# NIRVANALAN/LN3Diff

Hardware: AMD Instinct MI355X
Metric: 3D samples/sec (250-step DiT-L/2 + 256^2 triplane render) (higher is better)
Workload: dtype bf16; 1 GPU; BASELINE configs[1]: DiT-L/2 text-cond T23D, EulerEDM/LegacyDDPM-sigma 250 steps, CFG 6.5 (network batch 2B), batch 8 per GPU, VAE decode DiT2-L/2 + conv decoder, 40 views @ 256^2 (64+64 samples/ray); global_batch=8, views=40, res=256, parallelism=dp1 (independent samples per rank, no in-loop collective)

## Files before the change

### ln3diff_amd/csrc/gemm_bf16.hip

```cpp
#include <stdlib.h>
#include "common.h"
#include "../../include/ln3d.h"

#define BMF 128
#define BTK 128
#define BK 64
#define ROWB 144
#define TILEB (128 * ROWB)
#define GEMM_LDS (4 * TILEB)

#include "gemm_epi.h"

template <int EPI>
__global__ __launch_bounds__(256) void gemm_bf16_kernel(GemmP p) {
  extern __shared__ __attribute__((aligned(16))) char smem[];
  const int tid = threadIdx.x, lane = tid & 63, wid = tid >> 6;
  const int wf = wid >> 1, wt = wid & 1;
  const int l31 = lane & 31, hi = lane >> 5;

  const int nft = (p.N + BMF - 1) / BMF;
  const int ft = blockIdx.x % nft, tt = blockIdx.x / nft;
  const int f0 = ft * BMF, t0 = tt * BTK;

  const int c = tid & 7, r0 = tid >> 3;
  const bf16_t* wsrc[4]; const bf16_t* xsrc[4];
#pragma unroll
  for (int i = 0; i < 4; ++i) {
    int rf = f0 + r0 + 32 * i; rf = rf < p.N ? rf : p.N - 1;
    int rt = t0 + r0 + 32 * i; rt = rt < p.M ? rt : p.M - 1;
    wsrc[i] = p.W + (int64_t)rf * p.ldw + c * 8;
    xsrc[i] = p.X + (int64_t)rt * p.ldx + c * 8;
  }
  const int st_off = r0 * ROWB + c * 16;

  f32x16 acc[2][2];
#pragma unroll
  for (int i = 0; i < 2; ++i)
#pragma unroll
    for (int j = 0; j < 2; ++j)
#pragma unroll
      for (int r = 0; r < 16; ++r) acc[i][j][r] = 0.f;

  uint4 ra[4], rb[4];
  const int nk = p.K / BK;
#pragma unroll
  for (int i = 0; i < 4; ++i) {
    ra[i] = *reinterpret_cast<const uint4*>(wsrc[i]);
    rb[i] = *reinterpret_cast<const uint4*>(xsrc[i]);
  }
#pragma unroll
  for (int i = 0; i < 4; ++i) {
    *reinterpret_cast<uint4*>(smem + st_off + i * 32 * ROWB) = ra[i];
    *reinterpret_cast<uint4*>(smem + TILEB + st_off + i * 32 * ROWB) = rb[i];
  }
  __syncthreads();

  const int a_off = (wf * 64 + l31) * ROWB + hi * 16;
  const int b_off = TILEB + (wt * 64 + l31) * ROWB + hi * 16;

  auto mma_tile = [&](const char* base) {
#pragma unroll
    for (int ks = 0; ks < 4; ++ks) {
      bf16x8 a[2], b[2];
#pragma unroll
      for (int i = 0; i < 2; ++i) {
        a[i] = *reinterpret_cast<const bf16x8*>(base + a_off + i * 32 * ROWB + ks * 32);
        b[i] = *reinterpret_cast<const bf16x8*>(base + b_off + i * 32 * ROWB + ks * 32);
      }
#pragma unroll
      for (int i = 0; i < 2; ++i)
#pragma unroll
        for (int j = 0; j < 2; ++j)
          acc[i][j] = __builtin_amdgcn_mfma_f32_32x32x16_bf16(a[i], b[j], acc[i][j], 0, 0, 0);
    }
  };

  for (int kt = 0; kt + 1 < nk; ++kt) {
    const int buf = kt & 1;
    const int koff = (kt + 1) * BK;
    const uint4 na0 = *reinterpret_cast<const uint4*>(wsrc[0] + koff);
    const uint4 na1 = *reinterpret_cast<const uint4*>(wsrc[1] + koff);
    const uint4 na2 = *reinterpret_cast<const uint4*>(wsrc[2] + koff);
    const uint4 na3 = *reinterpret_cast<const uint4*>(wsrc[3] + koff);
    const uint4 nx0 = *reinterpret_cast<const uint4*>(xsrc[0] + koff);
    const uint4 nx1 = *reinterpret_cast<const uint4*>(xsrc[1] + koff);
    const uint4 nx2 = *reinterpret_cast<const uint4*>(xsrc[2] + koff);
    const uint4 nx3 = *reinterpret_cast<const uint4*>(xsrc[3] + koff);
    __builtin_amdgcn_sched_barrier(0);
    mma_tile(smem + buf * 2 * TILEB);
    __builtin_amdgcn_sched_barrier(0);
    char* nb = smem + (buf ^ 1) * 2 * TILEB + st_off;
    *reinterpret_cast<uint4*>(nb + 0 * 32 * ROWB) = na0;
    *reinterpret_cast<uint4*>(nb + 1 * 32 * ROWB) = na1;
    *reinterpret_cast<uint4*>(nb + 2 * 32 * ROWB) = na2;
    *reinterpret_cast<uint4*>(nb + 3 * 32 * ROWB) = na3;
    *reinterpret_cast<uint4*>(nb + TILEB + 0 * 32 * ROWB) = nx0;
    *reinterpret_cast<uint4*>(nb + TILEB + 1 * 32 * ROWB) = nx1;
    *reinterpret_cast<uint4*>(nb + TILEB + 2 * 32 * ROWB) = nx2;
    *reinterpret_cast<uint4*>(nb + TILEB + 3 * 32 * ROWB) = nx3;
    __syncthreads();
  }
  mma_tile(smem + ((nk - 1) & 1) * 2 * TILEB);

#pragma unroll
  for (int j = 0; j < 2; ++j) {
    const int tok = t0 + wt * 64 + j * 32 + l31;
    if (tok >= p.M) continue;
#pragma unroll
    for (int i = 0; i < 2; ++i) {
#pragma unroll
      for (int g = 0; g < 4; ++g) {
        const int fb = f0 + wf * 64 + i * 32 + 8 * g + 4 * hi;
        if (fb < p.N)
          epilogue4<EPI>(p, tok, fb, acc[i][j][4 * g + 0], acc[i][j][4 * g + 1], acc[i][j][4 * g + 2], acc[i][j][4 * g + 3]);
      }
    }
  }
}



template <int EPI, int NW, int WGT, int NI, int NJ>
__global__ __launch_bounds__(NW * 64, (NW == 4 && NI * NJ <= 6) ? 2 : NW / 4) void gemm_bf16_ring64_kernel(GemmP p) {
  constexpr int WGF = NW / WGT, BF = 32 * NI * WGF, BT = 32 * NJ * WGT;
  constexpr int WB = BF * 128, STAGEB = (BF + BT) * 128, NPW = (BF + BT) / 8 / NW;
  static_assert((BF + BT) / 8 % NW == 0, "DMA instructions must divide evenly over the waves");
  constexpr int NM = NI * NJ, NR = NI + NJ;
  static_assert(NM >= NR, "one fragment read per MFMA slot");
  extern __shared__ __attribute__((aligned(16))) char smem[];
  const int tid = threadIdx.x, lane = tid & 63;
  const int wid = __builtin_amdgcn_readfirstlane(tid >> 6);
  const int wf = wid / WGT, wt = wid % WGT;
  const int l31 = lane & 31, hi = lane >> 5;

  const int nft = (p.N + BF - 1) / BF, ntt = (p.M + BT - 1) / BT;
  const int ntiles = nft * ntt;
  int ft, tt;
  {
    const int b = blockIdx.x, xcd = b & 7, slot = b >> 3;
    if ((ntt & 7) == 0 && (nft & 3) == 0) {
      const int rows = ntt >> 3;
      const int g = slot / (rows * 4), rem = slot - g * rows * 4;
      ft = g * 4 + (rem & 3);
      tt = xcd * rows + (rem >> 2);
    } else {
      const int q = ntiles >> 3, r = ntiles & 7;
      const int tile = (xcd < r ? xcd * (q + 1) : r * (q + 1) + (xcd - r) * q) + slot;
      ft = tile % nft; tt = tile / nft;
    }
  }
  const int f0 = ft * BF, t0 = tt * BT;

  constexpr int NPWW = BF / 8 / NW, NPWX = BT / 8 / NW;
  static_assert(BF / 8 % NW == 0 && BT / 8 % NW == 0 && NPWW + NPWX == NPW, "row groups of both operands divide evenly over the waves");
  const int r8 = lane >> 3;
  const char* const Wb = reinterpret_cast<const char*>(p.W + (int64_t)f0 * p.ldw);
  const char* const Xb = reinterpret_cast<const char*>(p.X + (int64_t)t0 * p.ldx);
  uint32_t soff[NPW];
#pragma unroll
  for (int q = 0; q < NPW; ++q) {
    const int rt = 8 * (q < NPWW ? wid * NPWW + q : wid * NPWX + (q - NPWW)) + r8;
    const int chunk = (lane & 7) ^ ((rt >> 1) & 7);
    if (q < NPWW) {
      int r = f0 + rt; r = r < p.N ? r : p.N - 1;
      soff[q] = (uint32_t)(((int64_t)(r - f0) * p.ldw + chunk * 8) * 2);
    } else {
      int r = t0 + rt; r = r < p.M ? r : p.M - 1;
      soff[q] = (uint32_t)(((int64_t)(r - t0) * p.ldx + chunk * 8) * 2);
    }
  }
  const int dW0 = wid * NPWW * 1024, dX0 = WB + wid * NPWX * 1024;
  const uint32_t lds0 = (uint32_t)(uintptr_t)(lds_void_t*)smem;
#define Y_ISSUE1(s, q)                                                                                        \
  lds_dma16_s(((q) < NPWW ? Wb : Xb) + (int64_t)(s) * 128, soff[q],                                           \
              lds0 + ((s) & 1) * STAGEB + ((q) < NPWW ? dW0 + (q) * 1024 : dX0 + ((q) - NPWW) * 1024))

  const int key = (l31 >> 1) & 7;
  const int a_row = (wf * 32 * NI + l31) * 128;
  const int b_row = WB + (wt * 32 * NJ + l31) * 128;
#define Y_RDA(s, ks, i) (*reinterpret_cast<const bf16x8*>(smem + ((s) & 1) * STAGEB + a_row + (i) * 4096 + (((2 * (ks) + hi) ^ key) << 4)))
#define Y_RDB(s, ks, j) (*reinterpret_cast<const bf16x8*>(smem + ((s) & 1) * STAGEB + b_row + (j) * 4096 + (((2 * (ks) + hi) ^ key) << 4)))

  f32x16 acc[NI][NJ];
#pragma unroll
  for (int i = 0; i < NI; ++i)
#pragma unroll
    for (int j = 0; j < NJ; ++j)
#pragma unroll
      for (int r = 0; r < 16; ++r) acc[i][j][r] = 0.f;

  bf16x8 a0[NI], b0[NJ], a1[NI], b1[NJ];
  const int ns = p.K / 64;

  constexpr int XK = 2 * STAGEB, XKH = 96 * 128;
  if constexpr (EPI == LN3D_EPI_CROSS_ATTN) {
    static_assert(NI == 2 && NJ == 3 && WGT == 2 && (NW == 8 || NW == 4), "one head (64 features) per wave row: 256x192 (8 waves) or 128x192 (4 waves) tile");
    const int bsmp = t0 / p.tokens;
    const int nrows8 = (p.ctx_keys + 7) >> 3;
    const bf16_t* kc = (const bf16_t*)p.out1 + ((int64_t)bsmp * p.heads + (f0 >> 6)) * p.ctx_pad * 64;
    for (int idx = wid; idx < WGF * nrows8; idx += NW) {
      const int hh = idx / nrows8, j = idx - hh * nrows8;
      const int r = 8 * j + (lane >> 3);
      const bf16_t* src_k = kc + ((int64_t)hh * p.ctx_pad + r) * 64 + (((lane & 7) ^ ((r >> 1) & 7)) << 3);
      lds_dma16_v(src_k, lds0 + XK + hh * XKH + j * 1024);
    }
  }

#pragma unroll
  for (int q = 0; q < NPW; ++q) Y_ISSUE1(0, q);
  if (ns > 1) { _Pragma("unroll") for (int q = 0; q < NPW; ++q) Y_ISSUE1(1, q); }
  if (ns > 1) { asm volatile("s_waitcnt vmcnt(%0)" ::"n"(NPW) : "memory"); }
  else { asm volatile("s_waitcnt vmcnt(0)" ::: "memory"); }
  __builtin_amdgcn_s_barrier();
#pragma unroll
  for (int i = 0; i < NI; ++i) a0[i] = Y_RDA(0, 0, i);
#pragma unroll
  for (int j = 0; j < NJ; ++j) b0[j] = Y_RDB(0, 0, j);

#define Y_MMA(FA, FB, n) acc[(n) / NJ][(n) % NJ] = __builtin_amdgcn_mfma_f32_32x32x16_bf16(FA[(n) / NJ], FB[(n) % NJ], acc[(n) / NJ][(n) % NJ], 0, 0, 0)
  constexpr int D1 = (NPW + 1) / 2;
  constexpr int NLATE = NPW - D1;
#define Y_PHASE(CA, CB, NA, NB, s2, ks2, LATE, sd, L0, L1)                                                \
  _Pragma("unroll") for (int n = 0; n < NM; ++n) {                                                        \
    Y_MMA(CA, CB, n);                                                                                     \
    if (n < NI) NA[n] = Y_RDA(s2, ks2, n);                                                                \
    else if (n < NR) NB[n - NI] = Y_RDB(s2, ks2, n - NI);                                                 \
    if (LATE) {                                                                                           \
      _Pragma("unroll") for (int d = (L0); d < (L1); ++d)                                                 \
          if ((d - (L0)) * NM / ((L1) - (L0) > 0 ? (L1) - (L0) : 1) == n) Y_ISSUE1(sd, d);                \
    }                                                                                                     \
    __builtin_amdgcn_sched_barrier(0);                                                                    \
  }
  static_assert(NM - 1 >= NR, "one fragment read per MFMA slot behind the barrier");
  constexpr int LH = D1 + (NLATE + 1) / 2;
#define Y_STAGE(s, PREV, FILL, MORE)                                                                      \
  {                                                                                                       \
    Y_PHASE(a0, b0, a1, b1, s, 1, (PREV) && NLATE > 0, (s) + 1, D1, LH);                                  \
    Y_PHASE(a1, b1, a0, b0, s, 2, (PREV) && NLATE > 0, (s) + 1, LH, NPW);                                 \
    Y_PHASE(a0, b0, a1, b1, s, 3, false, 0, 0, 0);                                                        \
    _Pragma("unroll") for (int n = 0; n < NM; ++n) {                                                      \
      Y_MMA(a1, b1, n);                                                                                   \
      if (MORE && n == 0) {                                                                               \
        asm volatile("s_waitcnt vmcnt(0)" ::: "memory");                                                  \
        __builtin_amdgcn_s_waitcnt(0xC07F);                                                               \
        __builtin_amdgcn_s_barrier();                                                                     \
      }                                                                                                   \
      if (MORE) {                                                                                         \
        if (n >= 1 && n - 1 < NI) a0[n - 1] = Y_RDA((s) + 1, 0, n - 1);                                   \
        else if (n >= 1 && n - 1 < NR) b0[n - 1 - NI] = Y_RDB((s) + 1, 0, n - 1 - NI);                    \
      }                                                                                                   \
      if (FILL) {                                                                                         \
        _Pragma("unroll") for (int d = 0; d < D1; ++d)                                                    \
            if (1 + d * (NM - 1) / D1 == n) Y_ISSUE1((s) + 2, d);                                         \
      }                                                                                                   \
      __builtin_amdgcn_sched_barrier(0);                                                                  \
    }                                                                                                     \
  }
  __builtin_amdgcn_s_waitcnt(0xC07F);
  int s = 0;
  if (ns >= 3) {
    Y_STAGE(0, false, true, true);
    for (s = 1; s + 2 < ns; ++s) Y_STAGE(s, true, true, true);
    Y_STAGE(s, true, false, true);
    ++s;
  } else if (ns == 2) {
    Y_STAGE(0, false, false, true);
    s = 1;
  }
  constexpr bool kPre = EPI == LN3D_EPI_GATE_RES && NW <= 8 && NI % 2 == 0 && NI * NJ <= 6;
  float4 xpre[8];
  RunEpi<EPI> re_pre;
  bool have_pre = false;
  if constexpr (kPre) {
    const int fw0 = f0 + wf * 32 * NI, tw0 = t0 + wt * 32 * NJ;
    const bool full = (tw0 + 32 * NJ <= p.M) && (fw0 + 32 * NI <= p.N) && !((p.gate || p.rb) && p.gate_rows < 32);
    if (__builtin_amdgcn_readfirstlane(full ? 1 : 0)) {
      have_pre = true;
      const int rrow = lane >> 4, rc = lane & 15;
      re_pre.init(p, fw0 + 4 * rc, __builtin_amdgcn_readfirstlane(tw0), 0, 0, 0);
      const float* base = (const float*)p.out0 + (int64_t)(tw0 + rrow) * p.ldo + fw0 + 4 * rc;
#pragma unroll
      for (int it = 0; it < 8; ++it) xpre[it] = *reinterpret_cast<const float4*>(base + (int64_t)(4 * it) * p.ldo);
    }
  }
  Y_STAGE(s, false, false, false);

  if constexpr (EPI == LN3D_EPI_CROSS_ATTN) {
    const int bsmp = t0 / p.tokens;
    const int nkb = (p.ctx_keys + 63) >> 6, nkt = (p.ctx_keys + 31) >> 5;
    __builtin_amdgcn_s_barrier();
    {
      const bf16_t* vc = (const bf16_t*)p.out2 + ((int64_t)bsmp * p.heads + (f0 >> 6)) * 64 * p.ctx_pad;
      for (int idx = wid; idx < WGF * nkb * 8; idx += NW) {
        const int hh = idx / (nkb * 8), rem = idx - hh * nkb * 8, kb = rem >> 3, j = rem & 7;
        const int vrow = 8 * j + (lane >> 3);
        const bf16_t* src_v = vc + ((int64_t)hh * 64 + vrow) * p.ctx_pad + kb * 64 + (((lane & 7) ^ ((vrow >> 1) & 7)) << 3);
        lds_dma16_v(src_v, lds0 + (hh * 2 + kb) * 8192 + j * 1024);
      }
    }
    const int kkey = (l31 >> 1) & 7;
    const char* kbase = smem + XK + wf * XKH + l31 * 128;
    float inv[NJ];
    uint32_t pk[NJ][24];
#pragma unroll
    for (int j = 0; j < NJ; ++j) {
      f32x16 st[3];
#pragma unroll
      for (int kt = 0; kt < 3; ++kt)
#pragma unroll
        for (int r = 0; r < 16; ++r) st[kt][r] = 0.f;
#pragma unroll
      for (int sd = 0; sd < 4; ++sd) {
        union { uint32_t u[4]; bf16x8 v; } qb;
#pragma unroll
        for (int jj = 0; jj < 4; ++jj)
          qb.u[jj] = pack2bf(acc[sd >> 1][j][8 * (sd & 1) + 2 * jj], acc[sd >> 1][j][8 * (sd & 1) + 2 * jj + 1]);
#pragma unroll
        for (int kt = 0; kt < 3; ++kt)
          if (kt < nkt) {
            const bf16x8 kf = *reinterpret_cast<const bf16x8*>(kbase + kt * 32 * 128 + (((2 * sd + hi) ^ kkey) << 4));
            st[kt] = __builtin_amdgcn_mfma_f32_32x32x16_bf16(kf, qb.v, st[kt], 0, 0, 0);
          }
      }
      float mx = -3.0e38f;
#pragma unroll
      for (int kt = 0; kt < 3; ++kt)
#pragma unroll
        for (int r = 0; r < 16; ++r) {
          const int key = kt * 32 + 4 * hi + (r & 3) + 8 * (r >> 2);
          st[kt][r] = key < p.ctx_keys ? st[kt][r] : -3.0e38f;
          mx = fmaxf(mx, st[kt][r]);
        }
      mx = fmaxf(mx, __shfl_xor(mx, 32, 64));
      const float m = mx * p.ctx_scale_log2;
      float psum = 0.f;
#pragma unroll
      for (int kt = 0; kt < 3; ++kt)
#pragma unroll
        for (int r = 0; r < 16; ++r) {
          const float pv = __builtin_amdgcn_exp2f(fmaf(st[kt][r], p.ctx_scale_log2, -m));
          st[kt][r] = pv;
          psum += pv;
        }
      inv[j] = 1.0f / (psum + __shfl_xor(psum, 32, 64));
#pragma unroll
      for (int ks = 0; ks < 6; ++ks)
#pragma unroll
        for (int jj = 0; jj < 4; ++jj)
          pk[j][4 * ks + jj] = pack2bf(st[ks >> 1][8 * (ks & 1) + 2 * jj], st[ks >> 1][8 * (ks & 1) + 2 * jj + 1]);
    }
    asm volatile("s_waitcnt vmcnt(0)" ::: "memory");
    __builtin_amdgcn_s_barrier();
    const char* vbase = smem + (wf * 2) * 8192 + l31 * 128;
#pragma unroll
    for (int j = 0; j < NJ; ++j) {
      f32x16 oa[2];
#pragma unroll
      for (int dt = 0; dt < 2; ++dt)
#pragma unroll
        for (int r = 0; r < 16; ++r) oa[dt][r] = 0.f;
#pragma unroll
      for (int ks = 0; ks < 6; ++ks)
        if (ks < 2 * nkt) {
          union { uint32_t u[4]; bf16x8 v; } pb;
#pragma unroll
          for (int jj = 0; jj < 4; ++jj) pb.u[jj] = pk[j][4 * ks + jj];
#pragma unroll
          for (int dt = 0; dt < 2; ++dt) {
            const bf16x8 vf = *reinterpret_cast<const bf16x8*>(vbase + (ks >> 2) * 8192 + dt * 32 * 128 + (((2 * (ks & 3) + hi) ^ kkey) << 4));
            oa[dt] = __builtin_amdgcn_mfma_f32_32x32x16_bf16(vf, pb.v, oa[dt], 0, 0, 0);
          }
        }
#pragma unroll
      for (int dt = 0; dt < 2; ++dt)
#pragma unroll
        for (int r = 0; r < 16; ++r) acc[dt][j][r] = oa[dt][r] * inv[j];
    }
  }
  bool direct = false;
  if constexpr (EPI == LN3D_EPI_HEADS) {
    direct = (p.transpose_mask != 0) && (f0 + BF > 2 * p.heads * p.head_dim);
    if constexpr (NI == 2) {
      const int dm = p.heads * p.head_dim;
      if ((p.head_dim & 7) == 0 && (dm & 63) == 0 && (p.tokens & 31) == 0 && (p.M % p.tokens) == 0 && (p.N % 64) == 0) {
        const int fw0 = f0 + wf * 64;
        const int which = fw0 / dm;
        const bool tr = fw0 < p.N && ((p.transpose_mask >> which) & 1);
        const int HD = p.head_dim, DP = p.head_dim_pad;
        __builtin_amdgcn_s_barrier();
        if (tr) {
          char* stg = smem + wid * 8192;
          bf16_t* dst = (bf16_t*)(which == 0 ? p.out0 : (which == 1 ? p.out1 : p.out2));
          const int fr = lane >> 2, c = lane & 3;
          int64_t vrow[4];
#pragma unroll
          for (int it = 0; it < 4; ++it) {
            const int fr_ = fw0 - which * dm + 16 * it + fr;
            const int hh_ = fr_ / HD;
            vrow[it] = (int64_t)hh_ * DP + (fr_ - hh_ * HD);
          }
#pragma unroll
          for (int j = 0; j < NJ; ++j) {
            const int tb = __builtin_amdgcn_readfirstlane(t0 + wt * 32 * NJ + j * 32);
            if (tb >= p.M) break;
            const int tp = (l31 & ~12) | ((l31 & 4) << 1) | ((l31 & 8) >> 1);
#pragma unroll
            for (int i = 0; i < 2; ++i)
#pragma unroll
              for (int g = 0; g < 4; ++g)
#pragma unroll
                for (int e = 0; e < 4; ++e)
                  *reinterpret_cast<float*>(stg + (i * 32 + 8 * g + 4 * hi + e) * 128 + tp * 4) = acc[i][j][4 * g + e];
            const int b = tb / p.tokens, t = tb - b * p.tokens;
#pragma unroll
            for (int it = 0; it < 4; ++it) {
              const int f = 16 * it + fr;
              const float bv = p.bias ? p.bias[fw0 + f] : 0.f;
              const float4 v0 = *reinterpret_cast<const float4*>(stg + f * 128 + c * 32);
              const float4 v1 = *reinterpret_cast<const float4*>(stg + f * 128 + c * 32 + 16);
              uint4 o;
              o.x = pack2bf(v0.x + bv, v0.y + bv); o.y = pack2bf(v0.z + bv, v0.w + bv);
              o.z = pack2bf(v1.x + bv, v1.y + bv); o.w = pack2bf(v1.z + bv, v1.w + bv);
              *reinterpret_cast<uint4*>(dst + ((int64_t)b * p.heads * DP + vrow[it]) * p.tok_pad + t + 8 * c) = o;
            }
          }
        } else if (fw0 < p.N) {
          char* stg = smem + wid * 8192;
          bf16_t* dst = (bf16_t*)(which == 0 ? p.out0 : (which == 1 ? p.out1 : p.out2));
          const int r8 = lane >> 3, c8 = lane & 7;
          const int fc_ = fw0 - which * dm + 8 * c8;
          const int h = fc_ / HD, d8 = fc_ - h * HD;
          float4 b0 = make_float4(0.f, 0.f, 0.f, 0.f), b1 = b0;
          if (p.bias) { b0 = *reinterpret_cast<const float4*>(p.bias + fw0 + 8 * c8); b1 = *reinterpret_cast<const float4*>(p.bias + fw0 + 8 * c8 + 4); }
          const float* nw = (HD == 64 && DP == 64) ? (which == 0 ? p.hn0 : (which == 1 ? p.hn1 : nullptr)) : nullptr;
          float4 n0 = make_float4(1.f, 1.f, 1.f, 1.f), n1 = n0;
          if (nw) { n0 = *reinterpret_cast<const float4*>(nw + 8 * c8); n1 = *reinterpret_cast<const float4*>(nw + 8 * c8 + 4); }
#pragma unroll
          for (int j = 0; j < NJ; ++j) {
// ... 111 lines not shown
  const int64_t jstride = (int64_t)32 * p.ldo * 2;
#define P_STORE(j, k) *reinterpret_cast<uint4*>(pbase + (j) * jstride + ((k) >> 1) * 64 + ((k) & 1) * 32) = pend[((j) - 1) * 8 + (k)]
#define P_STOREQ(q) P_STORE(1 + (q) / 8, (q) % 8)
#define P_PHASE(CB, NB, rslot, ks2, RD, LATE, WL, XL, dslot, L0, L1, SJ, ZERO, SYNC, FILL, WF, XF, fslot)  \
  _Pragma("unroll") for (int n = 0; n < NM; ++n) {                                                        \
    if (ZERO) { P_MMA0(af, CB, n); } else { P_MMA(af, CB, n); }                                           \
    if ((SYNC) && n == 0) {                                                                               \
      if ((SJ) >= 0 && have) { asm volatile("s_waitcnt vmcnt(3)" ::: "memory"); }                         \
      else { asm volatile("s_waitcnt vmcnt(0)" ::: "memory"); }                                           \
      __builtin_amdgcn_s_waitcnt(0xC07F);                                                                 \
      __builtin_amdgcn_s_barrier();                                                                       \
    }                                                                                                     \
    if (RD) {                                                                                             \
      if ((n & 3) == 3) af[n >> 2] = P_RDA(rslot, ks2, n >> 2);                                           \
      else if (n == 1 || n == 2) NB[n - 1] = P_RDB(rslot, ks2, n - 1);                                    \
      else if (n == 4 || n == 5) NB[n - 2] = P_RDB(rslot, ks2, n - 2);                                    \
    }                                                                                                     \
    if (LATE) {                                                                                           \
      _Pragma("unroll") for (int d = (L0); d < (L1); ++d)                                                 \
          if ((d - (L0)) * NM / ((L1) - (L0)) == n) P_ISSUE(WL, XL, dslot, d);                            \
    }                                                                                                     \
    if (FILL) {                                                                                           \
      _Pragma("unroll") for (int d = 0; d < D1; ++d)                                                      \
          if (1 + d * (NM - 1) / D1 == n) P_ISSUE(WF, XF, fslot, d);                                      \
    }                                                                                                     \
    if (!(SYNC) && (SJ) >= 0 && (n & 3) == 1 && n < 12) { if (have) P_STOREQ(3 * ((SJ) < 0 ? 0 : (SJ)) + (n >> 2)); } \
    __builtin_amdgcn_sched_barrier(0);                                                                    \
  }
#define P_STAGE(slot, LATE, WL, XL, WF, XF, SJ, ZERO, PRE)                                                \
  {                                                                                                       \
    P_PHASE(b0, b1, slot, 1, true, LATE, WL, XL, (slot) ^ 1, D1, LH, -1, ZERO, false, false, WF, XF, slot);      \
    P_PHASE(b1, b0, slot, 2, true, LATE, WL, XL, (slot) ^ 1, LH, NPW, -1, false, false, false, WF, XF, slot);    \
    P_PHASE(b0, b1, slot, 3, true, false, WL, XL, (slot) ^ 1, 0, 1, SJ, false, false, false, WF, XF, slot);      \
    P_PHASE(b1, b0, (slot) ^ 1, 0, PRE, false, WL, XL, (slot) ^ 1, 0, 1, SJ, false, true, true, WF, XF, slot);   \
  }

  f32x16 acc[NI][NJ];
  bf16x8 af[NI], b0[NJ], b1[NJ];
  const int ns = p.K / 64;
  const int64_t ldw2 = p.ldw * 2, ldx2 = p.ldx * 2;

  int vb = blockIdx.x, ft, tt;
  tile_of(vb, ft, tt);
  const char* Wc = reinterpret_cast<const char*>(p.W) + (int64_t)ft * BF * ldw2;
  const char* Xc = reinterpret_cast<const char*>(p.X) + (int64_t)tt * BT * ldx2;
  int par = 0;
#pragma unroll
  for (int q = 0; q < NPW; ++q) P_ISSUE(Wc, Xc, 0, q);
#pragma unroll
  for (int q = 0; q < NPW; ++q) P_ISSUE(Wc + 128, Xc + 128, 1, q);
  const uint32_t boff = (uint32_t)lane * 16;
  if (p.bias) { if (wid == 0) lds_dma16_s(p.bias + ft * BF, boff, lds0 + BIASB); }
  else if (wid < 2) *reinterpret_cast<float4*>(smem + BIASB + wid * 1024 + lane * 16) = make_float4(0.f, 0.f, 0.f, 0.f);
  asm volatile("s_waitcnt vmcnt(0)" ::: "memory");
  __builtin_amdgcn_s_barrier();
  __builtin_amdgcn_s_waitcnt(0xC07F);

  for (;;) {
    const int vbn = vb + G;
    const bool has_next = vbn < ntiles;
    int ftn, ttn;
    tile_of(has_next ? vbn : vb, ftn, ttn);
    const char* Wn = reinterpret_cast<const char*>(p.W) + (int64_t)ftn * BF * ldw2;
    const char* Xn = reinterpret_cast<const char*>(p.X) + (int64_t)ttn * BT * ldx2;
#pragma unroll
    for (int i = 0; i < NI; ++i) af[i] = P_RDA(0, 0, i);
#pragma unroll
    for (int j = 0; j < NJ; ++j) b0[j] = P_RDB(0, 0, j);
    P_STAGE(0, false, Wc, Xc, Wc + 2 * 128, Xc + 2 * 128, 0, true, true);
    P_STAGE(1, true, Wc + 2 * 128, Xc + 2 * 128, Wc + 3 * 128, Xc + 3 * 128, 1, false, true);
    P_STAGE(0, true, Wc + 3 * 128, Xc + 3 * 128, Wc + 4 * 128, Xc + 4 * 128, 2, false, true);
    P_STAGE(1, true, Wc + 4 * 128, Xc + 4 * 128, Wc + 5 * 128, Xc + 5 * 128, 3, false, true);
    P_STAGE(0, true, Wc + 5 * 128, Xc + 5 * 128, Wc + 6 * 128, Xc + 6 * 128, 4, false, true);
    for (int s = 5; s + 3 < ns; s += 2) {
      P_STAGE(1, true, Wc + (s + 1) * 128, Xc + (s + 1) * 128, Wc + (s + 2) * 128, Xc + (s + 2) * 128, -1, false, true);
      P_STAGE(0, true, Wc + (s + 2) * 128, Xc + (s + 2) * 128, Wc + (s + 3) * 128, Xc + (s + 3) * 128, -1, false, true);
    }
    P_STAGE(1, true, Wc + (ns - 2) * 128, Xc + (ns - 2) * 128, Wc + (ns - 1) * 128, Xc + (ns - 1) * 128, 5, false, true);
    P_STAGE(0, true, Wc + (ns - 1) * 128, Xc + (ns - 1) * 128, Wn, Xn, 6, false, true);
    P_STAGE(1, true, Wn, Xn, Wn + 128, Xn + 128, 7, false, false);
#pragma unroll
    for (int d = D1; d < NPW; ++d) P_ISSUE(Wn + 128, Xn + 128, 1, d);
    if (p.bias && wid == 0) lds_dma16_s(p.bias + ftn * BF, boff, lds0 + BIASB + (par ^ 1) * 1024);

    {
      const float* bl = reinterpret_cast<const float*>(smem + BIASB + par * 1024) + wf * 128 + 4 * hi;
      char* const nbase = reinterpret_cast<char*>((bf16_t*)p.out0 + (int64_t)(tt * BT + wt * 128 + l31) * p.ldo + ft * BF + wf * 128 + 8 * hi);
#pragma unroll
      for (int i = 0; i < NI; ++i) {
        ln3d_f32x2 bq[2][4];
#pragma unroll
        for (int m = 0; m < 2; ++m) {
          const float4 bA = *reinterpret_cast<const float4*>(bl + i * 32 + 16 * m), bB = *reinterpret_cast<const float4*>(bl + i * 32 + 16 * m + 8);
          bq[m][0] = ln3d_f32x2{bA.x, bA.y}; bq[m][1] = ln3d_f32x2{bA.z, bA.w}; bq[m][2] = ln3d_f32x2{bB.x, bB.y}; bq[m][3] = ln3d_f32x2{bB.z, bB.w};
        }
#pragma unroll
        for (int j = 0; j < NJ; ++j) {
#pragma unroll
          for (int m = 0; m < 2; ++m) {
            ln3d_f32x2 v[4];
#pragma unroll
            for (int e = 0; e < 4; ++e) v[e] = ln3d_f32x2{acc[i][j][8 * m + 2 * e], acc[i][j][8 * m + 2 * e + 1]} + bq[m][e];
            if constexpr (EPI == LN3D_EPI_GELU_ERF) {
#pragma unroll
              for (int e = 0; e < 4; ++e) { float g0 = v[e].x, g1 = v[e].y; gelu_erf2(g0, g1); v[e] = ln3d_f32x2{g0, g1}; }
            }
            const uint32_t x0 = pack2bf(v[0].x, v[0].y), x1 = pack2bf(v[1].x, v[1].y), y0 = pack2bf(v[2].x, v[2].y), y1 = pack2bf(v[3].x, v[3].y);
            const auto r0 = __builtin_amdgcn_permlane32_swap(x0, y0, false, false);
            const auto r1 = __builtin_amdgcn_permlane32_swap(x1, y1, false, false);
            if (j == 0) *reinterpret_cast<uint4*>(nbase + i * 64 + m * 32) = make_uint4(r0[0], r1[0], r0[1], r1[1]);
            else pend[(j - 1) * 8 + i * 2 + m] = make_uint4(r0[0], r1[0], r0[1], r1[1]);
          }
          __builtin_amdgcn_sched_barrier(0);
        }
      }
      pbase = nbase;
      have = true;
    }
    if (!has_next) break;
    vb = vbn; ft = ftn; tt = ttn; Wc = Wn; Xc = Xn; par ^= 1;
  }
#pragma unroll
  for (int j = 1; j < NJ; ++j)
#pragma unroll
    for (int k = 0; k < 8; ++k) P_STORE(j, k);
  asm volatile("s_waitcnt vmcnt(0)" ::: "memory");
#undef P_ISSUE
#undef P_RDA
#undef P_RDB
#undef P_MMA
#undef P_STORE
#undef P_STOREQ
#undef P_MMA0
#undef P_PHASE
#undef P_STAGE
}

template <int EPI>
static int launch_p4(const GemmP& p, hipStream_t s) {
  constexpr int LDSB = 2 * (256 + 256) * 128 + 2048;
  static_assert(LDSB <= 163840, "ring + bias images");
  static AttrOnce attr_once;
  if (attr_once.need())
    (void)hipFuncSetAttribute(reinterpret_cast<const void*>(&gemm_bf16_p4_kernel<EPI>), hipFuncAttributeMaxDynamicSharedMemorySize, LDSB);
  const int ntiles = (p.N / 256) * (p.M / 256), cus = ln3d_stream_cus(s);
  hipLaunchKernelGGL((gemm_bf16_p4_kernel<EPI>), dim3(ntiles < cus ? ntiles : cus), dim3(256), LDSB, s, p);
  return ln3d_check_launch();
}
static bool p4_ok(const GemmP& p) {
  return (p.M % 256) == 0 && (p.N % 256) == 0 && (p.K % 128) == 0 && p.K >= 512 && (p.ldo % 8) == 0 &&
         ((uintptr_t)p.out0 & 15) == 0 && (!p.bias || ((uintptr_t)p.bias & 15) == 0);
}

template <int EPI, int NW, int WGT, int NI, int NJ>
static int launch_ring64(const GemmP& p, hipStream_t s) {
  constexpr int BF = 32 * NI * (NW / WGT), BT = 32 * NJ * WGT;
  constexpr int LDSB = 2 * (BF + BT) * 128 + (EPI == LN3D_EPI_CROSS_ATTN ? (NW / WGT) * 96 * 128 : 0);
  static_assert(2 * (BF + BT) * 128 >= NW * 8192 && LDSB <= 163840, "staging regions live in the ring");
  static AttrOnce attr_once;
  if (attr_once.need()) {
    (void)hipFuncSetAttribute(reinterpret_cast<const void*>(&gemm_bf16_ring64_kernel<EPI, NW, WGT, NI, NJ>),
                              hipFuncAttributeMaxDynamicSharedMemorySize, LDSB);
  }
  const int nft = (p.N + BF - 1) / BF, ntt = (p.M + BT - 1) / BT;
  hipLaunchKernelGGL((gemm_bf16_ring64_kernel<EPI, NW, WGT, NI, NJ>), dim3(nft * ntt), dim3(NW * 64), LDSB, s, p);
  return ln3d_check_launch();
}

template <int EPI>
static int launch(const GemmP& p, hipStream_t s) {
  static AttrOnce attr_once;
  if (attr_once.need()) {
    (void)hipFuncSetAttribute(reinterpret_cast<const void*>(&gemm_bf16_kernel<EPI>),
                        hipFuncAttributeMaxDynamicSharedMemorySize, GEMM_LDS);
  }
  const int nft = (p.N + BMF - 1) / BMF, ntt = (p.M + BTK - 1) / BTK;
  hipLaunchKernelGGL(gemm_bf16_kernel<EPI>, dim3(nft * ntt), dim3(256), GEMM_LDS, s, p);
  return ln3d_check_launch();
}

template <int EPI>
static int run_cfg(const GemmP& p, hipStream_t s, int cfg) {
  if constexpr (EPI == LN3D_EPI_CROSS_ATTN) return cfg == 14 ? launch_ring64<EPI, 4, 2, 2, 3>(p, s) : launch_ring64<EPI, 8, 2, 2, 3>(p, s);
  else
  switch (cfg) {
    case 7: return launch_ring64<EPI, 8, 4, 4, 2>(p, s);
    case 8: return launch_ring64<EPI, 8, 4, 2, 3>(p, s);
    case 9: return launch_ring64<EPI, 8, 2, 2, 3>(p, s);
    case 12: return launch_ring64<EPI, 12, 2, 2, 3>(p, s);
    case 14: return launch_ring64<EPI, 4, 2, 2, 3>(p, s);
    case 16:
      if constexpr (EPI == LN3D_EPI_BF16 || EPI == LN3D_EPI_GELU_ERF) { if (p4_ok(p)) return launch_p4<EPI>(p, s); }
      return launch_ring64<EPI, 8, 4, 4, 2>(p, s);
    case 13:
      if constexpr (EPI == LN3D_EPI_GATE_RES || EPI == LN3D_EPI_BF16 || EPI == LN3D_EPI_F32) return launch_ring64<EPI, 4, 2, 4, 4>(p, s);
      else return launch_ring64<EPI, 8, 4, 4, 2>(p, s);
    default: return launch<EPI>(p, s);
  }
}


static int g_gemm_forced = -2;
static int forced_cfg() {
  if (g_gemm_forced == -2) {
    const char* e = getenv("LN3D_GEMM_TILE");
    g_gemm_forced = !e ? -1 : (e[0] == 's' ? 0 : (e[0] == 'x' ? atoi(e + 1) : -1));
  }
  return g_gemm_forced;
}
extern "C" void ln3d_gemm_reload_env(void) { g_gemm_forced = -2; }
static int pick_cfg(int M, int N, bool head_aligned = false, hipStream_t s = nullptr, int K = 0, int epi = -1) {
  if (forced_cfg() >= 0) return forced_cfg();
  if (!(M >= 1536 && N >= 128)) return 0;
  static const struct { int cfg, bf, bt; float speed; } C[4] = {{7, 256, 256, 1.0f}, {12, 384, 192, 1.0f}, {9, 256, 192, 0.95f},
                                                               {8, 128, 384, 0.945f}};
  const int cus = ln3d_stream_cus(s);
  int best = 8; float best_cost = 1e30f; int64_t best_tiles = 0;
  for (int i = 0; i < 4; ++i) {
    if (head_aligned && C[i].cfg == 7) continue;
    const int64_t tiles = (int64_t)((N + C[i].bf - 1) / C[i].bf) * ((M + C[i].bt - 1) / C[i].bt);
    const float cost = (float)((tiles + cus - 1) / cus) * (float)(C[i].bf * C[i].bt) / C[i].speed;
    if (cost < best_cost) { best_cost = cost; best = C[i].cfg; best_tiles = tiles; }
  }
  if (best_tiles * 2 <= cus) {
    const int64_t t14 = (int64_t)((N + 127) / 128) * ((M + 191) / 192);
    if (t14 > best_tiles) best = 14;
  }
  if (best == 7 && K >= 2048 && best_tiles >= 2 * (int64_t)cus && (epi == LN3D_EPI_GATE_RES || epi == LN3D_EPI_BF16 || epi == LN3D_EPI_F32))
    best = 13;
  if ((epi == LN3D_EPI_BF16 || epi == LN3D_EPI_GELU_ERF) && (M % 256) == 0 && (N % 256) == 0 && (K % 128) == 0 && K >= 512) {
    const int64_t t = (int64_t)(N / 256) * (M / 256), rounds = (t + cus - 1) / cus;
    if (t >= 2 * (int64_t)cus && t * 100 >= rounds * cus * 85) best = 16;
  }
  return best;
}

extern "C" int ln3d_gemm_heads_norm_fusable(int M, int N, int tokens, int head_dim, int head_dim_pad) {
  if (head_dim_pad <= 0) head_dim_pad = head_dim;
  if (!(head_dim == 64 && head_dim_pad == 64 && tokens > 0 && (tokens & 31) == 0 && (M % tokens) == 0 && (N % 64) == 0)) return 0;
  const int cfg = pick_cfg(M, N, true);
  return (cfg == 8 || cfg == 9 || cfg == 12 || cfg == 14) ? 1 : 0;
}

extern "C" int ln3d_gemm_bf16(const ln3d_gemm_args* a, void* stream) {
  if (!a || !a->X || !a->W || !a->out0) return LN3D_ERR_BAD_ARG;
  if (a->M <= 0 || a->N <= 0 || a->K <= 0 || (a->K % BK) != 0 || (a->N % 4) != 0) return LN3D_ERR_BAD_ARG;
  if ((a->ldx % 8) != 0 || (a->ldw % 8) != 0) return LN3D_ERR_BAD_ARG;
  if (a->epilogue == LN3D_EPI_GATE_RES) {
    if (a->gate && ((a->gate_ld % 4) != 0 || ((uintptr_t)a->gate & 15) != 0)) return LN3D_ERR_BAD_ARG;
    if (a->res_bias && ((a->res_bias_ld % 4) != 0 || ((uintptr_t)a->res_bias & 15) != 0)) return LN3D_ERR_BAD_ARG;
    if ((a->gate || a->res_bias) && a->gate_rows <= 0) return LN3D_ERR_BAD_ARG;
  }
  GemmP p;
  p.X = (const bf16_t*)a->X; p.W = (const bf16_t*)a->W; p.bias = a->bias;
  p.ldx = a->ldx; p.ldw = a->ldw; p.ldo = a->ldo;
  p.M = a->M; p.N = a->N; p.K = a->K;
  p.out0 = a->out0; p.out1 = a->out1; p.out2 = a->out2;
  p.gate = a->gate; p.gate_rows = a->gate_rows > 0 ? a->gate_rows : 1; p.gate_ld = a->gate_ld;
  p.tokens = a->tokens; p.tok_pad = a->tok_pad; p.heads = a->heads; p.head_dim = a->head_dim;
  p.transpose_mask = a->transpose_mask;
  p.head_dim_pad = a->head_dim_pad > 0 ? a->head_dim_pad : a->head_dim;
  p.ctx_keys = a->ctx_keys; p.ctx_pad = a->ctx_pad; p.ctx_scale_log2 = a->ctx_scale * 1.4426950408889634f;
  p.hn0 = a->head_norm0; p.hn1 = a->head_norm1; p.hn_eps = a->head_norm_eps;
  p.rb = a->epilogue == LN3D_EPI_GATE_RES ? a->res_bias : nullptr; p.rb_ld = a->res_bias_ld;
  hipStream_t s = (hipStream_t)stream;
  const bool head_staged = a->epilogue == LN3D_EPI_HEADS && a->head_dim > 0 && (a->head_dim & 7) == 0 && a->heads > 0 &&
                           ((a->heads * a->head_dim) & 63) == 0 && a->tokens > 0 && (a->tokens & 31) == 0 && (a->M % a->tokens) == 0 &&
                           (a->N % 64) == 0;
  const int cfg = pick_cfg(a->M, a->N, head_staged, s, a->K, a->epilogue);
  switch (a->epilogue) {
    case LN3D_EPI_F32: return run_cfg<LN3D_EPI_F32>(p, s, cfg);
    case LN3D_EPI_BF16: return run_cfg<LN3D_EPI_BF16>(p, s, cfg);
    case LN3D_EPI_GELU_ERF: return run_cfg<LN3D_EPI_GELU_ERF>(p, s, cfg);
    case LN3D_EPI_GELU_TANH: return run_cfg<LN3D_EPI_GELU_TANH>(p, s, cfg);
    case LN3D_EPI_SILU: return run_cfg<LN3D_EPI_SILU>(p, s, cfg);
    case LN3D_EPI_QUICK_GELU: return run_cfg<LN3D_EPI_QUICK_GELU>(p, s, cfg);
    case LN3D_EPI_CROSS_ATTN:
      if (!a->out1 || !a->out2 || a->bias || a->head_dim != 64 || a->heads <= 0 || a->N != a->heads * 64 || a->tokens <= 0 ||
          (a->tokens % 192) != 0 || (a->M % a->tokens) != 0 || a->ctx_keys <= 0 || a->ctx_keys > 96 || a->ctx_pad < a->ctx_keys ||
          (a->ctx_pad % 64) != 0 || (a->N % 256) != 0)
        return LN3D_ERR_BAD_ARG;
      return run_cfg<LN3D_EPI_CROSS_ATTN>(p, s, ((int64_t)(a->N / 256) * ((a->M + 191) / 192) * 2 <= ln3d_stream_cus(s) && forced_cfg() != 9) ? 14 : 9);
    case LN3D_EPI_GATE_RES: return run_cfg<LN3D_EPI_GATE_RES>(p, s, cfg);
    case LN3D_EPI_F32_SILU:
      if (!a->out1) return LN3D_ERR_BAD_ARG;
      return run_cfg<LN3D_EPI_F32_SILU>(p, s, cfg);
    case LN3D_EPI_HEADS:
      if (a->tokens <= 0 || a->heads <= 0 || a->head_dim <= 0 || (a->head_dim % 4) != 0 || a->tok_pad < a->tokens)
        return LN3D_ERR_BAD_ARG;
      if ((a->head_norm0 || a->head_norm1) &&
          !((cfg == 8 || cfg == 9 || cfg == 12 || cfg == 14) && a->head_dim == 64 && p.head_dim_pad == 64 && (a->tokens & 31) == 0 &&
            (a->M % a->tokens) == 0 && (a->N % 64) == 0))
        return LN3D_ERR_UNSUPPORTED;
      return run_cfg<LN3D_EPI_HEADS>(p, s, cfg);
    default: return LN3D_ERR_UNSUPPORTED;
  }
}
```

Before: 2.711 samples/s.

## Add deeper multi-slot LDS ring to ring64 GEMM for small-grid gate-residual GEMMs

Generalizes the ring64 GEMM kernel's double-buffered LDS staging to a configurable NSLOT-deep ring (3 or 4 slots) with counted vmcnt waits. More K-tiles stay in flight per block. A new config 15 (4-wave 128x192 tile, 4 slots) is picked for gate-residual GEMMs whose tile count fits within one wave of CUs. The deeper prefetch is meant to hide global-memory latency when occupancy is low, at the cost of more LDS per block and more complex prologue/epilogue control.

```diff
diff --git a/ln3diff_amd/csrc/gemm_bf16.hip b/ln3diff_amd/csrc/gemm_bf16.hip
--- a/ln3diff_amd/csrc/gemm_bf16.hip
+++ b/ln3diff_amd/csrc/gemm_bf16.hip
@@ -120,7 +120,7 @@
 
 
 
-template <int EPI, int NW, int WGT, int NI, int NJ>
+template <int EPI, int NW, int WGT, int NI, int NJ, int NSLOT = 2>
 __global__ __launch_bounds__(NW * 64, (NW == 4 && NI * NJ <= 6) ? 2 : NW / 4) void gemm_bf16_ring64_kernel(GemmP p) {
   constexpr int WGF = NW / WGT, BF = 32 * NI * WGF, BT = 32 * NJ * WGT;
   constexpr int WB = BF * 128, STAGEB = (BF + BT) * 128, NPW = (BF + BT) / 8 / NW;
@@ -171,15 +171,15 @@
   }
   const int dW0 = wid * NPWW * 1024, dX0 = WB + wid * NPWX * 1024;
   const uint32_t lds0 = (uint32_t)(uintptr_t)(lds_void_t*)smem;
-#define Y_ISSUE1(s, q)                                                                                        \
+#define Y_ISSUE1(s, so, q)                                                                                    \
   lds_dma16_s(((q) < NPWW ? Wb : Xb) + (int64_t)(s) * 128, soff[q],                                           \
-              lds0 + ((s) & 1) * STAGEB + ((q) < NPWW ? dW0 + (q) * 1024 : dX0 + ((q) - NPWW) * 1024))
+              lds0 + (so) + ((q) < NPWW ? dW0 + (q) * 1024 : dX0 + ((q) - NPWW) * 1024))
 
   const int key = (l31 >> 1) & 7;
   const int a_row = (wf * 32 * NI + l31) * 128;
   const int b_row = WB + (wt * 32 * NJ + l31) * 128;
-#define Y_RDA(s, ks, i) (*reinterpret_cast<const bf16x8*>(smem + ((s) & 1) * STAGEB + a_row + (i) * 4096 + (((2 * (ks) + hi) ^ key) << 4)))
-#define Y_RDB(s, ks, j) (*reinterpret_cast<const bf16x8*>(smem + ((s) & 1) * STAGEB + b_row + (j) * 4096 + (((2 * (ks) + hi) ^ key) << 4)))
+#define Y_RDA(so, ks, i) (*reinterpret_cast<const bf16x8*>(smem + (so) + a_row + (i) * 4096 + (((2 * (ks) + hi) ^ key) << 4)))
+#define Y_RDB(so, ks, j) (*reinterpret_cast<const bf16x8*>(smem + (so) + b_row + (j) * 4096 + (((2 * (ks) + hi) ^ key) << 4)))
 
   f32x16 acc[NI][NJ];
 #pragma unroll
@@ -192,7 +192,7 @@
   bf16x8 a0[NI], b0[NJ], a1[NI], b1[NJ];
   const int ns = p.K / 64;
 
-  constexpr int XK = 2 * STAGEB, XKH = 96 * 128;
+  constexpr int XK = NSLOT * STAGEB, XKH = 96 * 128;
   if constexpr (EPI == LN3D_EPI_CROSS_ATTN) {
     static_assert(NI == 2 && NJ == 3 && WGT == 2 && (NW == 8 || NW == 4), "one head (64 features) per wave row: 256x192 (8 waves) or 128x192 (4 waves) tile");
     const int bsmp = t0 / p.tokens;
@@ -206,10 +206,16 @@
     }
   }
 
-#pragma unroll
-  for (int q = 0; q < NPW; ++q) Y_ISSUE1(0, q);
-  if (ns > 1) { _Pragma("unroll") for (int q = 0; q < NPW; ++q) Y_ISSUE1(1, q); }
-  if (ns > 1) { asm volatile("s_waitcnt vmcnt(%0)" ::"n"(NPW) : "memory"); }
+  static_assert(NSLOT >= 2 && NSLOT <= 4 && (NSLOT - 1) * NPW <= 63, "the counted waits fit the 6-bit vmcnt");
+#pragma unroll
+  for (int q = 0; q < NPW; ++q) Y_ISSUE1(0, 0, q);
+  if (ns > 1) { _Pragma("unroll") for (int q = 0; q < NPW; ++q) Y_ISSUE1(1, STAGEB, q); }
+  const bool ramp = NSLOT > 2 && ns > NSLOT;
+  if constexpr (NSLOT > 2) { if (!ramp && ns > 2) { _Pragma("unroll") for (int q = 0; q < NPW; ++q) Y_ISSUE1(2, 2 * STAGEB, q); } }
+  if constexpr (NSLOT > 3) { if (!ramp && ns > 3) { _Pragma("unroll") for (int q = 0; q < NPW; ++q) Y_ISSUE1(3, 3 * STAGEB, q); } }
+  if (NSLOT > 3 && !ramp && ns > 3) { asm volatile("s_waitcnt vmcnt(%0)" ::"n"(3 * NPW) : "memory"); }
+  else if (NSLOT > 2 && !ramp && ns > 2) { asm volatile("s_waitcnt vmcnt(%0)" ::"n"(2 * NPW) : "memory"); }
+  else if (ns > 1) { asm volatile("s_waitcnt vmcnt(%0)" ::"n"(NPW) : "memory"); }
   else { asm volatile("s_waitcnt vmcnt(0)" ::: "memory"); }
   __builtin_amdgcn_s_barrier();
 #pragma unroll
@@ -220,52 +226,92 @@
 #define Y_MMA(FA, FB, n) acc[(n) / NJ][(n) % NJ] = __builtin_amdgcn_mfma_f32_32x32x16_bf16(FA[(n) / NJ], FB[(n) % NJ], acc[(n) / NJ][(n) % NJ], 0, 0, 0)
   constexpr int D1 = (NPW + 1) / 2;
   constexpr int NLATE = NPW - D1;
-#define Y_PHASE(CA, CB, NA, NB, s2, ks2, LATE, sd, L0, L1)                                                \
+#define Y_PHASE(CA, CB, NA, NB, so2, ks2, LATE, sd, sod, L0, L1)                                          \
   _Pragma("unroll") for (int n = 0; n < NM; ++n) {                                                        \
     Y_MMA(CA, CB, n);                                                                                     \
-    if (n < NI) NA[n] = Y_RDA(s2, ks2, n);                                                                \
-    else if (n < NR) NB[n - NI] = Y_RDB(s2, ks2, n - NI);                                                 \
+    if (n < NI) NA[n] = Y_RDA(so2, ks2, n);                                                               \
+    else if (n < NR) NB[n - NI] = Y_RDB(so2, ks2, n - NI);                                                \
     if (LATE) {                                                                                           \
       _Pragma("unroll") for (int d = (L0); d < (L1); ++d)                                                 \
-          if ((d - (L0)) * NM / ((L1) - (L0) > 0 ? (L1) - (L0) : 1) == n) Y_ISSUE1(sd, d);                \
+          if ((d - (L0)) * NM / ((L1) - (L0) > 0 ? (L1) - (L0) : 1) == n) Y_ISSUE1(sd, sod, d);           \
     }                                                                                                     \
     __builtin_amdgcn_sched_barrier(0);                                                                    \
   }
   static_assert(NM - 1 >= NR, "one fragment read per MFMA slot behind the barrier");
   constexpr int LH = D1 + (NLATE + 1) / 2;
-#define Y_STAGE(s, PREV, FILL, MORE)                                                                      \
+#define Y_STAGE(so, son, sl, sop, sf, sof, PREV, FILL, MORE, WN)                                          \
   {                                                                                                       \
-    Y_PHASE(a0, b0, a1, b1, s, 1, (PREV) && NLATE > 0, (s) + 1, D1, LH);                                  \
-    Y_PHASE(a1, b1, a0, b0, s, 2, (PREV) && NLATE > 0, (s) + 1, LH, NPW);                                 \
-    Y_PHASE(a0, b0, a1, b1, s, 3, false, 0, 0, 0);                                                        \
+    Y_PHASE(a0, b0, a1, b1, so, 1, (PREV) && NLATE > 0, sl, sop, D1, LH);                                 \
+    Y_PHASE(a1, b1, a0, b0, so, 2, (PREV) && NLATE > 0, sl, sop, LH, NPW);                                \
+    Y_PHASE(a0, b0, a1, b1, so, 3, false, 0, 0, 0, 0);                                                    \
+    Y_LAST(son, sf, sof, FILL, MORE, WN);                                                                 \
+  }
+#define Y_LAST(son, sf, sof, FILL, MORE, WN)                                                              \
+  {                                                                                                       \
     _Pragma("unroll") for (int n = 0; n < NM; ++n) {                                                      \
       Y_MMA(a1, b1, n);                                                                                   \
       if (MORE && n == 0) {                                                                               \
-        asm volatile("s_waitcnt vmcnt(0)" ::: "memory");                                                  \
+        asm volatile("s_waitcnt vmcnt(%0)" ::"n"(WN) : "memory");                                         \
         __builtin_amdgcn_s_waitcnt(0xC07F);                                                               \
         __builtin_amdgcn_s_barrier();                                                                     \
       }                                                                                                   \
       if (MORE) {                                                                                         \
-        if (n >= 1 && n - 1 < NI) a0[n - 1] = Y_RDA((s) + 1, 0, n - 1);                                   \
-        else if (n >= 1 && n - 1 < NR) b0[n - 1 - NI] = Y_RDB((s) + 1, 0, n - 1 - NI);                    \
+        if (n >= 1 && n - 1 < NI) a0[n - 1] = Y_RDA(son, 0, n - 1);                                       \
+        else if (n >= 1 && n - 1 < NR) b0[n - 1 - NI] = Y_RDB(son, 0, n - 1 - NI);                        \
       }                                                                                                   \
       if (FILL) {                                                                                         \
         _Pragma("unroll") for (int d = 0; d < D1; ++d)                                                    \
-            if (1 + d * (NM - 1) / D1 == n) Y_ISSUE1((s) + 2, d);                                         \
+            if (1 + d * (NM - 1) / D1 == n) Y_ISSUE1(sf, sof, d);                                         \
       }                                                                                                   \
       __builtin_amdgcn_sched_barrier(0);                                                                  \
     }                                                                                                     \
   }
   __builtin_amdgcn_s_waitcnt(0xC07F);
-  int s = 0;
-  if (ns >= 3) {
-    Y_STAGE(0, false, true, true);
-    for (s = 1; s + 2 < ns; ++s) Y_STAGE(s, true, true, true);
-    Y_STAGE(s, true, false, true);
-    ++s;
-  } else if (ns == 2) {
-    Y_STAGE(0, false, false, true);
-    s = 1;
+  int s = 0, so = 0;
+  if constexpr (NSLOT == 2) {
+#define Y_SO2(s) (((s) & 1) * STAGEB)
+    if (ns >= 3) {
+      Y_STAGE(Y_SO2(0), Y_SO2(1), 1, Y_SO2(1), 2, Y_SO2(2), false, true, true, 0);
+      for (s = 1; s + 2 < ns; ++s) Y_STAGE(Y_SO2(s), Y_SO2((s) + 1), (s) + 1, Y_SO2((s) + 1), (s) + 2, Y_SO2((s) + 2), true, true, true, 0);
+      Y_STAGE(Y_SO2(s), Y_SO2((s) + 1), (s) + 1, Y_SO2((s) + 1), (s) + 2, Y_SO2((s) + 2), true, false, true, 0);
+      ++s;
+    } else if (ns == 2) {
+      Y_STAGE(Y_SO2(0), Y_SO2(1), 1, Y_SO2(1), 2, Y_SO2(2), false, false, true, 0);
+      s = 1;
+    }
+#undef Y_SO2
+  } else {
+    constexpr int RINGB = NSLOT * STAGEB;
+#define Y_SON (so + STAGEB == RINGB ? 0 : so + STAGEB)
+#define Y_SOP (so == 0 ? RINGB - STAGEB : so - STAGEB)
+#define Y_NEXT { ++s; so = Y_SON; }
+    if (ns > NSLOT) {
+      Y_PHASE(a0, b0, a1, b1, 0, 1, true, 2, 2 * STAGEB, 0, (NSLOT == 3 ? D1 : NPW));
+      Y_PHASE(a1, b1, a0, b0, 0, 2, true, NSLOT - 1, (NSLOT - 1) * STAGEB, (NSLOT == 3 ? D1 : 0), NPW);
+      Y_PHASE(a0, b0, a1, b1, 0, 3, false, 0, 0, 0, 0);
+      Y_LAST(STAGEB, NSLOT, 0, true, true, (NSLOT - 2) * NPW);
+      Y_NEXT;
+      while (s + NSLOT < ns) {
+        Y_STAGE(so, Y_SON, s + NSLOT - 1, Y_SOP, s + NSLOT, so, true, true, true, (NSLOT - 2) * NPW);
+        Y_NEXT;
+      }
+      Y_STAGE(so, Y_SON, s + NSLOT - 1, Y_SOP, s + NSLOT, so, true, false, true, (NSLOT - 2) * NPW);
+      Y_NEXT;
+    } else if (ns == NSLOT) {
+      Y_STAGE(so, Y_SON, s + NSLOT - 1, Y_SOP, s + NSLOT, so, false, false, true, (NSLOT - 2) * NPW);
+      Y_NEXT;
+    }
+    if constexpr (NSLOT > 3) {
+      if (ns > 2) {
+        Y_STAGE(so, Y_SON, s + NSLOT - 1, Y_SOP, s + NSLOT, so, false, false, true, NPW);
+        Y_NEXT;
+      }
+    }
+    if (ns > 1) {
+      Y_STAGE(so, Y_SON, s + NSLOT - 1, Y_SOP, s + NSLOT, so, false, false, true, 0);
+      Y_NEXT;
+    }
+#undef Y_NEXT
   }
   constexpr bool kPre = EPI == LN3D_EPI_GATE_RES && NW <= 8 && NI % 2 == 0 && NI * NJ <= 6;
   float4 xpre[8];
@@ -283,7 +329,7 @@
       for (int it = 0; it < 8; ++it) xpre[it] = *reinterpret_cast<const float4*>(base + (int64_t)(4 * it) * p.ldo);
     }
   }
-  Y_STAGE(s, false, false, false);
+  Y_STAGE((NSLOT == 2 ? ((s) & 1) * STAGEB : so), 0, 0, 0, 0, 0, false, false, false, 0);
 
   if constexpr (EPI == LN3D_EPI_CROSS_ATTN) {
     const int bsmp = t0 / p.tokens;
@@ -701,18 +747,18 @@
          ((uintptr_t)p.out0 & 15) == 0 && (!p.bias || ((uintptr_t)p.bias & 15) == 0);
 }
 
-template <int EPI, int NW, int WGT, int NI, int NJ>
+template <int EPI, int NW, int WGT, int NI, int NJ, int NSLOT = 2>
 static int launch_ring64(const GemmP& p, hipStream_t s) {
   constexpr int BF = 32 * NI * (NW / WGT), BT = 32 * NJ * WGT;
-  constexpr int LDSB = 2 * (BF + BT) * 128 + (EPI == LN3D_EPI_CROSS_ATTN ? (NW / WGT) * 96 * 128 : 0);
-  static_assert(2 * (BF + BT) * 128 >= NW * 8192 && LDSB <= 163840, "staging regions live in the ring");
+  constexpr int LDSB = NSLOT * (BF + BT) * 128 + (EPI == LN3D_EPI_CROSS_ATTN ? (NW / WGT) * 96 * 128 : 0);
+  static_assert(NSLOT * (BF + BT) * 128 >= NW * 8192 && LDSB <= 163840, "staging regions live in the ring");
   static AttrOnce attr_once;
   if (attr_once.need()) {
-    (void)hipFuncSetAttribute(reinterpret_cast<const void*>(&gemm_bf16_ring64_kernel<EPI, NW, WGT, NI, NJ>),
+    (void)hipFuncSetAttribute(reinterpret_cast<const void*>(&gemm_bf16_ring64_kernel<EPI, NW, WGT, NI, NJ, NSLOT>),
                               hipFuncAttributeMaxDynamicSharedMemorySize, LDSB);
   }
   const int nft = (p.N + BF - 1) / BF, ntt = (p.M + BT - 1) / BT;
-  hipLaunchKernelGGL((gemm_bf16_ring64_kernel<EPI, NW, WGT, NI, NJ>), dim3(nft * ntt), dim3(NW * 64), LDSB, s, p);
+  hipLaunchKernelGGL((gemm_bf16_ring64_kernel<EPI, NW, WGT, NI, NJ, NSLOT>), dim3(nft * ntt), dim3(NW * 64), LDSB, s, p);
   return ln3d_check_launch();
 }
 
@@ -730,7 +776,8 @@
 
 template <int EPI>
 static int run_cfg(const GemmP& p, hipStream_t s, int cfg) {
-  if constexpr (EPI == LN3D_EPI_CROSS_ATTN) return cfg == 14 ? launch_ring64<EPI, 4, 2, 2, 3>(p, s) : launch_ring64<EPI, 8, 2, 2, 3>(p, s);
+  if constexpr (EPI == LN3D_EPI_CROSS_ATTN)
+    return cfg == 15 ? launch_ring64<EPI, 4, 2, 2, 3, 3>(p, s) : (cfg == 14 ? launch_ring64<EPI, 4, 2, 2, 3>(p, s) : launch_ring64<EPI, 8, 2, 2, 3>(p, s));
   else
   switch (cfg) {
     case 7: return launch_ring64<EPI, 8, 4, 4, 2>(p, s);
@@ -738,6 +785,7 @@
     case 9: return launch_ring64<EPI, 8, 2, 2, 3>(p, s);
     case 12: return launch_ring64<EPI, 12, 2, 2, 3>(p, s);
     case 14: return launch_ring64<EPI, 4, 2, 2, 3>(p, s);
+    case 15: return launch_ring64<EPI, 4, 2, 2, 3, 4>(p, s);
     case 16:
       if constexpr (EPI == LN3D_EPI_BF16 || EPI == LN3D_EPI_GELU_ERF) { if (p4_ok(p)) return launch_p4<EPI>(p, s); }
       return launch_ring64<EPI, 8, 4, 4, 2>(p, s);
@@ -758,6 +806,7 @@
   return g_gemm_forced;
 }
 extern "C" void ln3d_gemm_reload_env(void) { g_gemm_forced = -2; }
+static bool deep_ring_epi(int epi) { return epi == LN3D_EPI_GATE_RES; }
 static int pick_cfg(int M, int N, bool head_aligned = false, hipStream_t s = nullptr, int K = 0, int epi = -1) {
   if (forced_cfg() >= 0) return forced_cfg();
   if (!(M >= 1536 && N >= 128)) return 0;
@@ -774,6 +823,7 @@
   if (best_tiles * 2 <= cus) {
     const int64_t t14 = (int64_t)((N + 127) / 128) * ((M + 191) / 192);
     if (t14 > best_tiles) best = 14;
+    if (best == 14 && t14 <= cus && deep_ring_epi(epi)) best = 15;
   }
   if (best == 7 && K >= 2048 && best_tiles >= 2 * (int64_t)cus && (epi == LN3D_EPI_GATE_RES || epi == LN3D_EPI_BF16 || epi == LN3D_EPI_F32))
     best = 13;
@@ -788,7 +838,7 @@
   if (head_dim_pad <= 0) head_dim_pad = head_dim;
   if (!(head_dim == 64 && head_dim_pad == 64 && tokens > 0 && (tokens & 31) == 0 && (M % tokens) == 0 && (N % 64) == 0)) return 0;
   const int cfg = pick_cfg(M, N, true);
-  return (cfg == 8 || cfg == 9 || cfg == 12 || cfg == 14) ? 1 : 0;
+  return (cfg == 8 || cfg == 9 || cfg == 12 || cfg == 14 || cfg == 15) ? 1 : 0;
 }
 
 extern "C" int ln3d_gemm_bf16(const ln3d_gemm_args* a, void* stream) {
@@ -829,7 +879,13 @@
           (a->tokens % 192) != 0 || (a->M % a->tokens) != 0 || a->ctx_keys <= 0 || a->ctx_keys > 96 || a->ctx_pad < a->ctx_keys ||
           (a->ctx_pad % 64) != 0 || (a->N % 256) != 0)
         return LN3D_ERR_BAD_ARG;
-      return run_cfg<LN3D_EPI_CROSS_ATTN>(p, s, ((int64_t)(a->N / 256) * ((a->M + 191) / 192) * 2 <= ln3d_stream_cus(s) && forced_cfg() != 9) ? 14 : 9);
+      {
+        const int f = forced_cfg(), cus = ln3d_stream_cus(s);
+        if (f == 9 || f == 14 || f == 15) return run_cfg<LN3D_EPI_CROSS_ATTN>(p, s, f);
+        const int64_t t9 = (int64_t)(a->N / 256) * ((a->M + 191) / 192);
+        if (t9 * 2 > cus) return run_cfg<LN3D_EPI_CROSS_ATTN>(p, s, 9);
+        return run_cfg<LN3D_EPI_CROSS_ATTN>(p, s, 14);
+      }
     case LN3D_EPI_GATE_RES: return run_cfg<LN3D_EPI_GATE_RES>(p, s, cfg);
     case LN3D_EPI_F32_SILU:
       if (!a->out1) return LN3D_ERR_BAD_ARG;
@@ -838,7 +894,7 @@
       if (a->tokens <= 0 || a->heads <= 0 || a->head_dim <= 0 || (a->head_dim % 4) != 0 || a->tok_pad < a->tokens)
         return LN3D_ERR_BAD_ARG;
       if ((a->head_norm0 || a->head_norm1) &&
-          !((cfg == 8 || cfg == 9 || cfg == 12 || cfg == 14) && a->head_dim == 64 && p.head_dim_pad == 64 && (a->tokens & 31) == 0 &&
+          !((cfg == 8 || cfg == 9 || cfg == 12 || cfg == 14 || cfg == 15) && a->head_dim == 64 && p.head_dim_pad == 64 && (a->tokens & 31) == 0 &&
             (a->M % a->tokens) == 0 && (a->N % 64) == 0))
         return LN3D_ERR_UNSUPPORTED;
       return run_cfg<LN3D_EPI_HEADS>(p, s, cfg);
```

Measured after the change: 2.727 samples/s, median of 6. Within noise of the previous version (+0.6%).
